# buckbaskin/parakeet_slam

Hardware: AMD Instinct MI355X
Metric: particle*landmark EKF updates/sec (whole filter step) (higher is better)
Workload: dtype f64

## Files before the change

include/parakeet_slam.h:

```cpp
#ifndef PARAKEET_SLAM_H_
#define PARAKEET_SLAM_H_

#include <stddef.h>
#include <stdint.h>

#ifdef __cplusplus
extern "C" {
#endif
#if defined(__GNUC__)
#pragma GCC visibility push(default)
#endif

#define PK_ABI_VERSION 1

typedef enum pk_status {
  PK_OK = 0,
  PK_ERR_INVALID = -1,
  PK_ERR_HIP = -2,
  PK_ERR_STATE = -3,
  PK_ERR_UNSUPPORTED = -4,
  PK_ERR_NOMEM = -5
} pk_status;

#define PK_LANDMARK_POTENTIAL 0x40000000
// ... 102 lines not shown
int pk_shard_adopt_local_dev(pk_filter* f, int32_t rank);
int pk_shard_adopt_remote_dev(pk_filter* f, int32_t rank, const void* dev_recv, int64_t n_received);
int pk_motion_range(pk_filter* f, double v, double w, double dt, uint64_t seed, uint64_t draw, int64_t p0, int64_t p1);
int pk_staged_takes_regs(pk_filter* f);
int pk_observe_staged_range(pk_filter* f, int32_t fresh, int64_t p0, int64_t p1, int32_t first, int32_t last);

int pk_shard_state_dev(pk_filter* f, double* dev_out);
int pk_shard_plan_balanced_dev(pk_filter* f, const double* dev_global_state, int64_t global_particles, const double* dev_gmax,
                               int32_t weight_domain, double u, int32_t world, int32_t rank, int64_t* dev_table);
int pk_shard_pack_balanced_dev(pk_filter* f, const int64_t* table, int32_t world, int32_t rank, void* dev_buf);
int pk_shard_adopt_balanced_dev(pk_filter* f, const int64_t* table, int32_t world, int32_t rank, const void* dev_recv,
                                int64_t n_received, int32_t mode);
int pk_shard_pack_balanced_loop_dev(pk_filter* f, int64_t keep, int64_t a0, int64_t a1, void* dev_buf);
int pk_shard_download_logical(pk_filter* f, int64_t* logical);
int pk_shard_upload_logical(pk_filter* f, const int64_t* logical);
int pk_shard_download_balanced_plan(pk_filter* f, int64_t* rel, int64_t* Hl, int32_t* alive);
int pk_shard_reset_placement(pk_filter* f);
int pk_shard_download_balanced_offspring(pk_filter* f, int64_t global_particles, int64_t* H);
int pk_shard_balanced_errors(pk_filter* f, int64_t* count);

#define PK_PROBE_LEN 79
int pk_probe(int32_t device, const double pose[3], const double mean[5], const double cov[25],
             const double blob[4], const double Qt[16], double* out);

int pk_enable_timing(pk_filter* f, int32_t mask);
int pk_reset_timings(pk_filter* f);
int pk_timings(pk_filter* f, double ms[PK_T_COUNT], int64_t launches[PK_T_COUNT]);
int pk_observe_bytes(const pk_filter* f, int32_t num_blobs, int64_t* algorithmic, int64_t* moved);
enum {
  PK_ROUTE_NONE = 0,
  PK_ROUTE_KNOWN_IDS = 1,
  PK_ROUTE_ML_GENERAL = 2,
  PK_ROUTE_ML_HANDOFF = 3,
  PK_ROUTE_ML_SWEEP = 4,
  PK_ROUTE_ML_FUSED = 5,
  PK_ROUTE_ML_REGS = 6,
  PK_ROUTE_DENSE = 8,
  PK_ROUTE_ML_PUB_BIG = 9,
};
int pk_observe_route(const pk_filter* f);
int pk_download_sources(pk_filter* f, int32_t* src);
int pk_observe_flagged(pk_filter* f, int64_t* flagged, int64_t* cand_overflow);
int pk_observe_retry_rows(pk_filter* f, int64_t* wanted, int64_t* capacity);
int pk_observe_published(pk_filter* f, int32_t* published);
int pk_observe_pub_stats(pk_filter* f, int64_t stats[6]);
int pk_observe_flags(pk_filter* f, uint8_t* flags);
// ... 16 lines not shown
```

parakeet_slam_amd/_lib.py:

```python
from __future__ import annotations

import ctypes as C
import os

import numpy as np

HERE = os.path.dirname(os.path.abspath(__file__))
LIB_PATH = os.path.join(HERE, "libparakeet_slam.so")

PK_OK = 0
PK_ERR_INVALID, PK_ERR_HIP, PK_ERR_STATE, PK_ERR_UNSUPPORTED, PK_ERR_NOMEM = -1, -2, -3, -4, -5
PK_WEIGHTS_LINEAR, PK_WEIGHTS_LOG = 0, 1
PK_LANDMARK_POTENTIAL = 0x40000000
PK_T_NAMES = ("motion", "assoc", "observe", "weights", "resample", "summary", "materialise")
PK_T_COUNT = len(PK_T_NAMES)
PK_PROBE_LEN = 79
PK_ABI_VERSION = 1

_dp = C.POINTER(C.c_double)
_ip = C.POINTER(C.c_int32)
_lp = C.POINTER(C.c_int64)
_bp = C.POINTER(C.c_uint8)
_h = C.c_void_p

# ... 48 lines not shown
    "pk_shard_adopt_dev": (C.c_int, [_h, C.c_int32, C.c_void_p, C.c_int64]),
    "pk_shard_local_span_dev": (C.c_int, [_h, C.c_void_p]),
    "pk_shard_adopt_local_dev": (C.c_int, [_h, C.c_int32]),
    "pk_shard_adopt_remote_dev": (C.c_int, [_h, C.c_int32, C.c_void_p, C.c_int64]),
    "pk_shard_state_dev": (C.c_int, [_h, C.c_void_p]),
    "pk_shard_plan_balanced_dev": (C.c_int, [_h, C.c_void_p, C.c_int64, C.c_void_p, C.c_int32, C.c_double, C.c_int32, C.c_int32,
                                             C.c_void_p]),
    "pk_shard_pack_balanced_dev": (C.c_int, [_h, _lp, C.c_int32, C.c_int32, C.c_void_p]),
    "pk_shard_adopt_balanced_dev": (C.c_int, [_h, _lp, C.c_int32, C.c_int32, C.c_void_p, C.c_int64, C.c_int32]),
    "pk_shard_pack_balanced_loop_dev": (C.c_int, [_h, C.c_int64, C.c_int64, C.c_int64, C.c_void_p]),
    "pk_shard_download_logical": (C.c_int, [_h, _lp]),
    "pk_shard_reset_placement": (C.c_int, [_h]),
    "pk_shard_upload_logical": (C.c_int, [_h, _lp]),
    "pk_shard_download_balanced_plan": (C.c_int, [_h, _lp, _lp, _ip]),
    "pk_shard_download_balanced_offspring": (C.c_int, [_h, C.c_int64, _lp]),
    "pk_shard_balanced_errors": (C.c_int, [_h, _lp]),
    "pk_motion_range": (C.c_int, [_h, C.c_double, C.c_double, C.c_double, C.c_uint64, C.c_uint64, C.c_int64, C.c_int64]),
    "pk_staged_takes_regs": (C.c_int, [_h]),
    "pk_observe_staged_range": (C.c_int, [_h, C.c_int32, C.c_int64, C.c_int64, C.c_int32, C.c_int32]),
    "pk_particle_bytes": (C.c_int64, [_h]),
    "pk_pack_particles": (C.c_int, [_h, _lp, C.c_int64, C.c_void_p]),
    "pk_adopt_particles": (C.c_int, [_h, _lp, C.c_void_p, C.c_int64]),
    "pk_probe": (C.c_int, [C.c_int32, _dp, _dp, _dp, _dp, _dp, _dp]),
    "pk_enable_timing": (C.c_int, [_h, C.c_int32]),
    "pk_reset_timings": (C.c_int, [_h]),
    "pk_timings": (C.c_int, [_h, _dp, _lp]),
    "pk_observe_bytes": (C.c_int, [_h, C.c_int32, _lp, _lp]),
    "pk_observe_route": (C.c_int, [_h]),
    "pk_download_sources": (C.c_int, [_h, _ip]),
    "pk_observe_flagged": (C.c_int, [_h, _lp, _lp]),
    "pk_observe_retry_rows": (C.c_int, [_h, _lp, _lp]),
    "pk_grow_enable": (C.c_int, [_h, C.c_int32, C.c_int32, C.c_double]),
    "pk_grow_download": (C.c_int, [_h, C.c_int64, C.c_int64, _ip, _dp, _ip]),
    "pk_grow_upload": (C.c_int, [_h, C.c_int64, C.c_int64, _ip, _dp, _ip]),
    "pk_grow_shape": (C.c_int, [_h, C.POINTER(C.c_int32), C.POINTER(C.c_int32), C.POINTER(C.c_int32)]),
    "pk_observe_published": (C.c_int, [_h, C.POINTER(C.c_int32)]),
    "pk_observe_flags": (C.c_int, [_h, _bp]),
    "pk_observe_pub_stats": (C.c_int, [_h, _lp]),
    "pk_rng_create_numpy": (C.c_int, [C.c_uint32, C.POINTER(_h)]),
    "pk_rng_create_python": (C.c_int, [C.c_uint32, C.POINTER(_h)]),
    "pk_rng_destroy": (C.c_int, [_h]),
    "pk_rng_standard_normal": (C.c_int, [_h, C.c_int64, _dp]),
    "pk_rng_random": (C.c_int, [_h, C.c_int64, _dp]),
}


# ... 390 lines not shown
        return {k: (float(ms[i]), int(n[i])) for i, k in enumerate(PK_T_NAMES)}

    def observe_bytes(self, num_blobs):
        a = C.c_int64()
        m = C.c_int64()
        check(self._lib.pk_observe_bytes(self._h, int(num_blobs), C.byref(a), C.byref(m)))
        return int(a.value), int(m.value)


def probe(pose, mean, cov, blob, Qt=None, device=0):
    lib = load()
    Qt = 0.1 * np.identity(4) if Qt is None else Qt
    out = np.empty(PK_PROBE_LEN, dtype=np.float64)
    check(lib.pk_probe(int(device), dptr(f64(pose, (3,))), dptr(f64(mean, (5,))), dptr(f64(cov, (25,))),
                       dptr(f64(blob, (4,))), dptr(f64(Qt, (16,))), dptr(out)))
    return dict(
        probability_of_match=out[0], prob_position_match=out[1], closest_point=out[2:4].copy(),
        prob_color_match=out[4], zhat=out[5:9].copy(), H0=out[9:11].copy(), Q=out[11:27].reshape(4, 4).copy(),
        K=out[27:47].reshape(5, 4).copy(), weight=out[47], new_mean=out[48:53].copy(),
        new_cov=out[53:78].reshape(5, 5).copy(), log_weight=out[78],
    )


class HostRng(object):

    def __init__(self, seed, kind="numpy"):
        self._lib = load()
        self._h = _h()
        fn = self._lib.pk_rng_create_numpy if kind == "numpy" else self._lib.pk_rng_create_python
        check(fn(int(seed) & 0xFFFFFFFF, C.byref(self._h)))

    def standard_normal(self, n):
        out = np.empty(int(n), dtype=np.float64)
        check(self._lib.pk_rng_standard_normal(self._h, int(n), dptr(out)))
        return out

    def random(self, n=None):
        out = np.empty(1 if n is None else int(n), dtype=np.float64)
        check(self._lib.pk_rng_random(self._h, out.size, dptr(out)))
        return float(out[0]) if n is None else out

    def __del__(self):
        try:
            if self._h.value:
                self._lib.pk_rng_destroy(self._h)
                self._h = _h()
# ... 3 lines not shown
```

parakeet_slam_amd/csrc/pk_api.hip:

```cpp
#include <hip/hip_runtime.h>

#include <cmath>
#include <cstdarg>
#include <cstdio>
#include <cstring>
#include <new>
#include <string>
#include <vector>

#include "../../include/parakeet_slam.h"
#include "pk_kernels.hpp"

using namespace pk;

extern "C" {
int pk_download_landmarks(pk_filter* f, int64_t p0, int64_t p1, double* means, double* covs, int32_t* counts);
int pk_upload_landmarks(pk_filter* f, int64_t p0, int64_t p1, const double* means, const double* covs, const int32_t* counts);
}

#ifdef PK_STAMPS
namespace pk { void debug_read_stamps(unsigned long long* out, bool reset); void debug_read_fused_stamps(unsigned long long* out, bool reset); void debug_read_regs_stamps(unsigned long long* out, bool reset); void debug_read_pub_stamps(unsigned long long* out, bool reset); void debug_read_pub_wave_stamps(unsigned long long* out, bool reset); }
#endif

namespace {
// ... 2605 lines not shown
  PK_HIP(hipSetDevice(device));
  double in[55];
  memcpy(in, pose, 3 * 8);
  memcpy(in + 3, mean, 5 * 8);
  memcpy(in + 8, cov, 25 * 8);
  memcpy(in + 33, blob, 4 * 8);
  memcpy(in + 37, Qt, 16 * 8);
  blob_directions(blob, 1, in + 53);
  double* dev = nullptr;
  PK_HIP(hipMalloc((void**)&dev, (55 + PK_PROBE_LEN) * sizeof(double)));
  hipError_t e = hipMemcpy(dev, in, sizeof(in), hipMemcpyHostToDevice);
  if (e == hipSuccess) {
    if (dense)
      launch_probe_dense(nullptr, dev, dev + 55);
    else
      launch_probe(nullptr, dev, dev + 55);
    e = hipMemcpy(out, dev + 55, PK_PROBE_LEN * sizeof(double), hipMemcpyDeviceToHost);
  }
  (void)hipFree(dev);
  if (e != hipSuccess) return fail(PK_ERR_HIP, "pk_probe: %s", hipGetErrorString(e));
  return PK_OK;
}

#ifdef PK_STAMPS
__attribute__((visibility("default"))) int pk_debug_pub_wave_stamps(unsigned long long* out, int reset) {
  pk::debug_read_pub_wave_stamps(out, reset != 0);
  return PK_OK;
}
__attribute__((visibility("default"))) int pk_debug_stamps(unsigned long long* out, int reset) {
  pk::debug_read_stamps(out, reset != 0);
  pk::debug_read_fused_stamps(out + 16, reset != 0);
  pk::debug_read_regs_stamps(out + 32, reset != 0);
  pk::debug_read_pub_stamps(out + 48, reset != 0);
  return PK_OK;
}
#endif

int pk_enable_timing(pk_filter* f, int32_t on) {
  if (!f) return fail(PK_ERR_INVALID, "pk_enable_timing: NULL handle");
  int rc;
  if ((rc = use_device(f))) return rc;
  if ((rc = drain_timings(f))) return rc;
  f->timing_mask = on < 0 ? 0xffffffffu : (uint32_t)on;
  return PK_OK;
}
int pk_reset_timings(pk_filter* f) {
// ... 106 lines not shown
```

parakeet_slam_amd/csrc/pk_device.hpp:

```cpp
#pragma once
#include <hip/hip_runtime.h>

#include <cfloat>
#include <climits>
#include <cstring>
#include <type_traits>

#include "pk_kernels.hpp"
#include "pk_math.hpp"

namespace pk {

constexpr int kWave = 64;
constexpr int kObsThreads = 256;
constexpr int kRedBlocks = 1024;

__device__ __forceinline__ void lds_barrier() { asm volatile("s_waitcnt lgkmcnt(0)\n\ts_barrier" ::: "memory"); }

#ifdef PK_STAMPS
#define PK_STAMP(var) \
  unsigned long long var; \
  asm volatile("s_memtime %0\n\ts_waitcnt lgkmcnt(0)" : "=s"(var)::"memory");
#else
#define PK_STAMP(var)
#endif

__device__ __forceinline__ double wave_sum(double v) {
#pragma unroll
  for (int off = 32; off > 0; off >>= 1) v += __shfl_xor(v, off, kWave);
  return v;
}
__device__ __forceinline__ double wave_max(double v) {
#pragma unroll
  for (int off = 32; off > 0; off >>= 1) v = fmax(v, __shfl_xor(v, off, kWave));
  return v;
}

template <int NW>
__device__ __forceinline__ double block_sum(double v, double* lds ) {
  v = wave_sum(v);
  const int wave = threadIdx.x / kWave, lane = threadIdx.x % kWave;
  __syncthreads();
  if (lane == 0) lds[wave] = v;
  __syncthreads();
  double t = lds[0];
#pragma unroll
  for (int i = 1; i < NW; ++i) t += lds[i];
  return t;
}
template <int NW>
__device__ __forceinline__ double block_sum_lds_only(double v, double* lds , int tid) {
  v = wave_sum(v);
// ... 96 lines not shown
```

parakeet_slam_amd/csrc/pk_k_motion.hip:

```cpp
#include "pk_device.hpp"
#include "pk_philox.hpp"

namespace pk {

__global__ void __launch_bounds__(256) k_motion(double* __restrict__ x, double* __restrict__ y,
                                                double* __restrict__ h, int64_t P, double v, double w,
                                                double dt, double sd, double sh,
                                                const double* __restrict__ z, uint64_t seed,
                                                uint64_t draw, int64_t goff, int motion_blocks,
                                                uint4* __restrict__ up_dst, const uint4* __restrict__ up_src,
                                                int64_t up_n16, const int64_t* __restrict__ logical,
                                                double* __restrict__ pose_part) {
  __shared__ double red[4];
  if ((int)blockIdx.x >= motion_blocks) {
    const int64_t nb = (int64_t)gridDim.x - motion_blocks;
    for (int64_t i = (int64_t)(blockIdx.x - motion_blocks) * blockDim.x + threadIdx.x; i < up_n16; i += nb * blockDim.x)
      up_dst[i] = up_src[i];
    return;
  }
  int64_t i = (int64_t)blockIdx.x * blockDim.x + threadIdx.x;
  if (i >= P && pose_part == nullptr) return;
  double px = 0.0, py = 0.0, ps = 0.0, pc = 0.0;
  if (i < P) {
  double z0, z1, z2;
// ... 226 lines not shown
  out[50] = g.mr;
  out[51] = g.mg;
  out[52] = g.mb;
  double* S = out + 53;
  S[0] = g.pxx;
  S[1] = g.pxy;
  S[5] = g.pxy;
  S[6] = g.pyy;
  S[12] = g.crr;
  S[13] = g.crg;
  S[14] = g.crb;
  S[17] = g.crg;
  S[18] = g.cgg;
  S[19] = g.cgb;
  S[22] = g.crb;
  S[23] = g.cgb;
  S[24] = g.cbb;
  out[78] = lw;
}
void launch_probe(hipStream_t s, const double* in_dev, double* out_dev) {
  hipLaunchKernelGGL(k_probe, dim3(1), dim3(64), 0, s, in_dev, out_dev);
}

}
```

parakeet_slam_amd/csrc/pk_k_step_pub.hip:

```cpp
#include <type_traits>

#include "pk_device.hpp"
#include "pk_pub_math.hpp"
#include "pk_pub_layout.hpp"

namespace pk {

#ifndef PK_PUB_ABLATE
#define PK_PUB_ABLATE 0
#endif

typedef double Double2 __attribute__((ext_vector_type(2)));
typedef int Int2 __attribute__((ext_vector_type(2)));

__device__ __forceinline__ double pose_scalar(const double* a, int64_t p) {
  return ((const __attribute__((address_space(4))) double*)a)[p];
}
__device__ __forceinline__ int32_t regs_source_pub(const int32_t* src, int64_t p) {
  return ((const __attribute__((address_space(4))) int32_t*)src)[p];
}

struct PubArgs {
  SlotSource ss;
  unsigned char* map_dst;
// ... 634 lines not shown
        for (int r = kMid; r < SLOTS; ++r) {
          contenders += v[h][r] < pub_inf() ? 1 : 0;
          close |= v[h][r] != best[h] && v[h][r] - best[h] < 1e-7;
        }
      }
      doubt |= close || (contenders >= 2 && best[h] > 1350.0);
    }
#pragma unroll
    for (int h = 0; h < TWO; ++h) {
      unsigned we = kRankMajor ? g[h] : offs[h] + wr[h];
      if constexpr (kRankMajor) we += wr[h] == 0u ? 0u : wr[h] == 1u ? G : rb[wr[h]];
      pub[best[h] < pub_inf() ? we : dump] = best[h] < pub_inf() ? pub_marker() : pub_inf();
    }
  }
  if (doubt) *flag = 1;
}

__device__ __forceinline__ void pub_take(PubSlots& q, const double* pub, unsigned dump) {
  const unsigned sw[kPubSlots] = {q.s[0], q.s[1], q.s[2], q.s[3]};
  double m[kPubSlots];
#pragma unroll
  for (int s = 0; s < kPubSlots; ++s) {
    const unsigned e = sw[s] >> 16;
    m[s] = pub[e == 0xFFFFu ? dump : e];
  }
#pragma unroll
  for (int s = 0; s < kPubSlots; ++s) {
    const unsigned e = sw[s] >> 16;
    const bool pos = ((q.st >> (4 * s)) & 1u) != 0u;
    if (pos && (e == 0xFFFFu || m[s] == pub_marker())) q.st |= 4u << (4 * s);
  }
}

#ifndef PK_DIAG_LOG_PER_UPDATE
#define PK_PROD_PTR(p_) (&(p_))
#else
#define PK_PROD_PTR(p_) ((double*)nullptr)
#endif
__device__ __forceinline__ void pub_fold_norms(double& acc, double& prod, bool last) {
#ifndef PK_DIAG_LOG_PER_UPDATE
  if (last || __ballot(!(prod > 1e-150 && prod < 1e150)) != 0ull) {
    acc -= 0.25 * log_few_ulp(prod);
    prod = 1.0;
  }
#else
  (void)acc;
  (void)prod;
// ... 122 lines not shown
  (void)hipDeviceSynchronize();
  (void)hipMemcpyFromSymbol(out, HIP_SYMBOL(pk_pstamp_acc), sizeof(unsigned long long) * 16);
  if (reset) {
    unsigned long long z[16] = {0};
    (void)hipMemcpyToSymbol(HIP_SYMBOL(pk_pstamp_acc), z, sizeof(z));
  }
}
#else
#define PK_PSTAMP(slot, a, b)
#endif

typedef const __attribute__((address_space(4))) PubArgs* PubArgsPtr;
__device__ __forceinline__ PubArgsPtr pub_args_now(PubArgsPtr rp) {
  asm volatile("" : "+s"(rp));
  return rp;
}
__device__ __forceinline__ SlotSource pub_slot_source(PubArgsPtr R) {
  return SlotSource{R->ss.map, R->ss.slot_bytes, R->ss.alt, R->ss.alt_stride, R->ss.alt_off};
}
__device__ __forceinline__ Noise<double> pub_noise(PubArgsPtr R) {
  return Noise<double>{R->qt.q00, R->qt.rr, R->qt.rg, R->qt.rb, R->qt.gg, R->qt.gb, R->qt.bb, R->qt.diag};
}

#ifdef PK_DIAG_NO_XCD_RUNS
__device__ __forceinline__ int64_t pub_walk_first(int64_t p_begin, int64_t) { return p_begin + blockIdx.x; }
__device__ __forceinline__ int64_t pub_walk_stride() { return (int64_t)gridDim.x; }
__device__ __forceinline__ int64_t pub_walk_limit(int64_t, int64_t p_end) { return p_end; }
#else
__device__ __forceinline__ int64_t pub_walk_first(int64_t p_begin, int64_t p_end) {
  const unsigned g = gridDim.x, b = blockIdx.x;
  if ((g & 7u) != 0u) return p_begin + b;
  const int64_t chunk = (p_end - p_begin + 7) / 8;
  return p_begin + (int64_t)(b & 7u) * chunk + (int64_t)(b >> 3);
}
__device__ __forceinline__ int64_t pub_walk_stride() { return (gridDim.x & 7u) != 0u ? (int64_t)gridDim.x : (int64_t)(gridDim.x >> 3); }
__device__ __forceinline__ int64_t pub_walk_limit(int64_t p_begin, int64_t p_end) {
  const unsigned g = gridDim.x, b = blockIdx.x;
  if ((g & 7u) != 0u) return p_end;
  const int64_t chunk = (p_end - p_begin + 7) / 8, e = p_begin + (int64_t)((b & 7u) + 1u) * chunk;
  return e < p_end ? e : p_end;
}
#endif
template <int NP, int THREADS>
__global__ void __launch_bounds__(THREADS, THREADS == 256 ? 3 : 1) k_step_pub(PubArgs a_unused) {
  constexpr int kPubThreads = THREADS, kPubWaves = THREADS / kWave;
  extern __shared__ __align__(16) unsigned char smem[];
  __shared__ double red[2][kPubWaves];
  __shared__ int wg_flag[2];
  constexpr bool kPerm = NP == 2 && THREADS == 512;
  __shared__ unsigned short s_perm[kPerm ? 2 * kPubOctets : 1];
  __shared__ unsigned s_rb[kCandSlots];
  constexpr int kUnmWords = THREADS == kPubSmallThreads ? 32 : 96;
  __shared__ unsigned s_ubits[kUnmWords];
#define PK_PUB_L0(q_, t_) (!kPerm ? 2 * kPubThreads * (q_) + 2 * (t_) : (int)(((lw >> (16 + 8 * (q_))) & 0xFFu) << 4) + 2 * ((t_)&7))
  PubArgsPtr rp = (PubArgsPtr)__builtin_amdgcn_kernarg_segment_ptr();
  const int tid0 = threadIdx.x;
  int B, Lp, L, ecap;
  {
    PubArgsPtr R = pub_args_now(rp);
    if (*R->skip != 0u) return;
    B = R->B;
    Lp = R->Lp;
    L = R->L;
    ecap = R->ecap;
  }
  const unsigned Bp = ((unsigned)B + 15u) & ~15u;
  const unsigned o_pub = Bp * 48u, o_binfo = o_pub + ((unsigned)ecap + 2u) * 8u, o_order = o_binfo + Bp * 4u, o_any = o_order + Bp * 2u;
  const unsigned o_imm = o_any + 2u * (Bp + 16u);
  const unsigned o_bnd = o_imm + (unsigned)kPubImmBytes;
  const unsigned dump = (unsigned)ecap, anydump = Bp;
  unsigned G;
  {
    const int tid = tid0;
    PubArgsPtr R = pub_args_now(rp);
    {
      const uint4* gf = R->far;
      float2* bnd = reinterpret_cast<float2*>(smem + o_bnd);
      for (int i = tid; i < Lp; i += kPubThreads) {
        float2 v = make_float2(-3.0e38f, 0.f);
        if (gf) {
          const uint4 hdr = gf[2 * (size_t)i];
          if (hdr.z != 0u) v = make_float2(__uint_as_float(hdr.x), __uint_as_float(hdr.y));
        }
        bnd[i] = v;
      }
    }
    double* ex = reinterpret_cast<double*>(smem);
    const double* gex = R->exact;
// ... 3 lines not shown
    const unsigned* gb = R->glist;
    const unsigned short* go = R->order;
    G = gb[B];
    for (int i = tid; i < B; i += kPubThreads) {
      glist[i] = (unsigned)i < G ? gb[i] : 0u;
      order[i] = go[i];
    }
    for (unsigned i = (unsigned)tid; i < 2u * (Bp + 16u) / 4u; i += kPubThreads) reinterpret_cast<unsigned*>(smem + o_any)[i] = 0u;
    const unsigned char* gi = R->immutable;
    for (int i = tid; i < Lp; i += kPubThreads) smem[o_imm + (unsigned)i] = i < L ? gi[i] : (unsigned char)0;
    if constexpr (kPerm) {
      if (tid < 2 * kPubOctets) s_perm[tid] = reinterpret_cast<const unsigned short*>(gb + B + 1)[tid];
    }
    if (tid < kCandSlots) s_rb[tid] = gb[B + 1 + kPubTailWords + tid];
    for (int i = tid; i < kUnmWords; i += kPubThreads) s_ubits[i] = 0u;
    if (tid == 0) {
      wg_flag[0] = 0;
      wg_flag[1] = 0;
    }
  }
  __syncthreads();

  int64_t prev = -1;
  int cur = 0;
  int32_t nsrc;
  {
    PubArgsPtr R = pub_args_now(rp);
    const int64_t p0 = pub_walk_first(R->p_begin, R->P), pl = pub_walk_limit(R->p_begin, R->P);
    nsrc = regs_source_pub(R->src, p0 < pl ? p0 : pl - 1);
  }
#ifdef PK_STAMPS
  unsigned long long pst[12] = {0, 0, 0, 0, 0, 0, 0, 0, 0, 0, 0, 0};
#endif
#define PK_PUB_ROW(q_, field, F)                                                                  \
  {                                                                                               \
    const Double2 v_ = *reinterpret_cast<const Double2*>(sf_ + (size_t)F * Lp + lbq_);            \
    S[2 * (q_)].field = v_.x;                                                                     \
    S[2 * (q_) + 1].field = v_.y;                                                                 \
  }
#define PK_PUB_LOAD_MEANS(q_, sslot_, lb_)                                                        \
  {                                                                                               \
    const double* sf_ = reinterpret_cast<const double*>(sslot_);                                  \
    const int lbq_ = (lb_);                                                                       \
    PK_PUB_ROW(q_, mx, F_MX)                                                                      \
    PK_PUB_ROW(q_, my, F_MY)                                                                      \
    PK_PUB_ROW(q_, mr, F_MR)                                                                      \
// ... 70 lines not shown
      tid = (int)(lw & 0xFFFFu);
    }
    double* ex = reinterpret_cast<double*>(smem);
    double* pub = reinterpret_cast<double*>(smem + o_pub);
    const unsigned* glist = reinterpret_cast<const unsigned*>(smem + o_binfo);
    const unsigned short* order = reinterpret_cast<const unsigned short*>(smem + o_order);
    unsigned char* anyc = smem + o_any + (unsigned)cur * (Bp + 16u);
    PubSlots Q[2 * NP];
    double pse[2 * NP];
    bool done;
    PK_STAMP(s0)
#ifdef PK_STAMPS
    unsigned long long s3 = s0;
#endif
    {
      PubArgsPtr R = pub_args_now(rp);
      const int64_t Pn = pub_walk_limit(R->p_begin, R->P);
      done = p >= Pn;
      const int64_t pc = done ? Pn - 1 : p;
      {
        const SlotSource ss = pub_slot_source(R);
        const unsigned char* sslot = ss.at(nsrc);
        const double sx = pose_scalar(R->x, pc), sy = pose_scalar(R->y, pc), sh = pose_scalar(R->h, pc);
        int lbase[NP];
#pragma unroll
        for (int q = 0; q < NP; ++q) lbase[q] = min(PK_PUB_L0(q, tid), Lp - 2);
        uint4 cref[2 * NP], ccw[2 * NP], cew[2 * NP];
        auto request_cand = [&](int q) {
          PubArgsPtr R2 = pub_args_now(rp);
#ifdef PK_DIAG_TAIL_LISTS
          const int lc = lbase[q];
#else
          const int lc = min(PK_PUB_L0(q, tid), Lp);
#endif
          const uint4* cr = R2->cand + 2 * (size_t)lc;
          const uint4* er = R2->erec + lc;
          cref[2 * q] = cr[0];
          ccw[2 * q] = cr[1];
          cref[2 * q + 1] = cr[2];
          ccw[2 * q + 1] = cr[3];
          cew[2 * q] = er[0];
          cew[2 * q + 1] = er[1];
        };
        request_cand(0);
        asm volatile("" ::: "memory");
        {
// ... 84 lines not shown
        if (!done) {
          do_pair(std::integral_constant<int, 0>{});
          if constexpr (NP > 1) {
            PK_PUB_LOAD_MEANS(1, sslot, lbase[1])
            request_cand(NP - 1);
            {
              asm volatile("" ::: "memory");
              PubArgsPtr R7 = pub_args_now(rp);
              PK_PUB_LOAD_COVS(1, sslot, R7->count_off, lbase[1])
            }
            do_pair(std::integral_constant<int, 1>{});
          }
        }
        PK_STAMP(s2)
        PK_PSTAMP(1, s1, s2)
#ifdef PK_STAMPS
        s3 = s2;
#endif
      }
    }
    lds_barrier();
    PK_STAMP(s4)
    PK_PSTAMP(3, s3, s4)
    if (prev >= 0 && tid == 0) {
      PubArgsPtr R = pub_args_now(rp);
      double tot = red[cur ^ 1][0];
#pragma unroll
      for (int i = 1; i < kPubWaves; ++i) tot += red[cur ^ 1][i];
      double* logw = R->logw;
      const double w = (R->reset ? 0.0 : logw[prev]) + tot;
      logw[prev] = w;
      unsigned long long* gk = R->gmax_key;
      if (gk) atomicMax(gk + (prev & (kGmaxKeys - 1)), double_to_key(w));
      R->src[prev] = (int32_t)prev;
    }
    if (done) break;
    prev = -1;
    double acc;
    {
      int nun = 0;
      for (unsigned w = (unsigned)tid; w < Bp / 4u; w += kPubThreads) {
        const unsigned v = reinterpret_cast<const unsigned*>(anyc)[w];
#pragma unroll
        for (int b = 0; b < 4; ++b) nun += ((int)(4 * w + b) < B && ((v >> (8 * b)) & 0xFFu) == 0u) ? 1 : 0;
      }
      acc = (double)nun * Consts<double>::log_no_match;
      unsigned* anyn = reinterpret_cast<unsigned*>(smem + o_any + (unsigned)(cur ^ 1) * (Bp + 16u));
      for (unsigned w = (unsigned)tid; w < Bp / 4u; w += kPubThreads) anyn[w] = 0u;
      if (tid == 0) wg_flag[cur ^ 1] = 0;
    }
    if (pub_args_now(rp)->unm != nullptr) pub_note_unmatched<THREADS>(tid, anyc, order, B, Bp, s_ubits);
    if (PK_PUB_ABLATE < 2) pub_settle_blobs<THREADS>(tid, glist, G, pub, dump, &wg_flag[cur], s_rb);
    PK_STAMP(s5)
    PK_PSTAMP(4, s4, s5)
    lds_barrier();
    {
      PubArgsPtr Ru = pub_args_now(rp);
      if (Ru->unm != nullptr) pub_store_unmatched<THREADS>(tid, s_ubits, Ru->unm + (size_t)p * Ru->unm_words, Ru->unm_words);
    }
#pragma unroll
    for (int i = 0; i < 2 * NP; ++i)
      if (PK_PUB_ABLATE < 2) pub_take(Q[i], pub, dump);
    lds_barrier();
    PK_STAMP(s6)
    PK_PSTAMP(5, s5, s6)
    if (wg_flag[cur] && PK_PUB_ABLATE == 0) {
      if (tid == 0) {
        PubArgsPtr R = pub_args_now(rp);
        R->pflag_out[p] = 1;
        atomicAdd(R->n_flagged, 1u);
      }
      {
        PubArgsPtr R6 = pub_args_now(rp);
        const unsigned char* ns = pub_slot_source(R6).at(nsrc);
        const int coff = R6->count_off;
#pragma unroll
        for (int q = 0; q < kPipe; ++q) PK_PUB_LOAD_PAIR(q, ns, coff, min(PK_PUB_L0(q, tid), Lp - 2))
      }
      continue;
    }
    {
      PubArgsPtr R = pub_args_now(rp);
      if (tid == 0) R->pflag_out[p] = 0;
      const Noise<double> qt = pub_noise(R);
      const double sx = pose_scalar(R->x, p), sy = pose_scalar(R->y, p);
      unsigned char* dslot = R->map_dst + (size_t)p * R->ss.slot_bytes;
      double* df = reinterpret_cast<double*>(dslot);
      int* dc = reinterpret_cast<int*>(dslot + R->count_off);
// ... 168 lines not shown

#define PK_BIG_FIRST(R_) pub_walk_first((R_)->p_begin, (R_)->P)
#define PK_BIG_STRIDE() pub_walk_stride()
#define PK_BIG_LIMIT(R_) pub_walk_limit((R_)->p_begin, (R_)->P)
template <int NCH>
__global__ void __launch_bounds__(kPubThreads) k_step_pub_big(PubArgs a_unused) {
  extern __shared__ __align__(16) unsigned char smem[];
  __shared__ double red[2][kPubThreads / kWave];
  __shared__ int wg_flag[2];
  __shared__ unsigned short s_bperm[kPubBigPlaces];
  __shared__ unsigned s_rb[kPubBigSlots];
  __shared__ unsigned s_novf[2];
  __shared__ unsigned s_ubits[kPubUnmWords];
#define PK_BIG_L0(q_, t_) ((int)(16u * (unsigned)s_bperm[kPubOctets * (q_) + ((t_) >> 3)]) + 2 * ((t_)&7))
  constexpr int kPubWaves = kPubThreads / kWave;
#ifdef PK_DIAG_BIG_FRONT_TO_BACK
  constexpr bool kBack = false;
#else
  constexpr bool kBack = NCH < 6;
#endif
  PubArgsPtr rp = (PubArgsPtr)__builtin_amdgcn_kernarg_segment_ptr();
  const int tid0 = threadIdx.x;
  int B, Lp, L, ecap;
  {
    PubArgsPtr R = pub_args_now(rp);
    if (*R->skip != 0u) return;
    B = R->B;
    Lp = R->Lp;
    L = R->L;
    ecap = R->ecap;
  }
  const unsigned Bp = ((unsigned)B + 15u) & ~15u;
  const unsigned o_glist = ((unsigned)ecap + 2u) * 8u, o_any = o_glist + Bp * 4u;
  const unsigned dump = (unsigned)ecap, anydump = Bp;
  unsigned G;
  unsigned ovf0, n_places;
  {
    const int tid = tid0;
    PubArgsPtr R = pub_args_now(rp);
    unsigned* glist = reinterpret_cast<unsigned*>(smem + o_glist);
    const unsigned* gb = R->glist;
    G = gb[B];
    const unsigned E = R->stats[0];
    ovf0 = (E + 1u) & ~1u;
    n_places = (unsigned)ecap > ovf0 ? ((unsigned)ecap - ovf0) / 2u : 0u;
    if (n_places > 0xFFFEu) n_places = 0xFFFEu;
    for (int i = tid; i < B; i += kPubThreads) glist[i] = (unsigned)i < G ? gb[i] : 0u;
    for (unsigned i = (unsigned)tid; i < 2u * (Bp + 16u) / 4u; i += kPubThreads) reinterpret_cast<unsigned*>(smem + o_any)[i] = 0u;
    if (tid < kPubBigPlaces) s_bperm[tid] = reinterpret_cast<const unsigned short*>(gb + B + 1)[2 * kPubOctets + tid];
    if (tid < kPubBigSlots) s_rb[tid] = gb[B + 1 + kPubTailWords + tid];
    for (int i = tid; i < kPubUnmWords; i += kPubThreads) s_ubits[i] = 0u;
    if (tid == 0) {
      wg_flag[0] = 0;
      wg_flag[1] = 0;
// ... 17 lines not shown
    PK_BIG_LOAD(SA, SB, mb, F_MB, lb_)                                                                \
    asm volatile("" ::: "memory");                                                                    \
    PK_BIG_LOAD(SA, SB, pxx, F_PXX, lb_)                                                              \
    PK_BIG_LOAD(SA, SB, pxy, F_PXY, lb_)                                                              \
    PK_BIG_LOAD(SA, SB, pyy, F_PYY, lb_)                                                              \
    PK_BIG_LOAD(SA, SB, crr, F_CRR, lb_)                                                              \
    PK_BIG_LOAD(SA, SB, crg, F_CRG, lb_)                                                              \
    PK_BIG_LOAD(SA, SB, crb, F_CRB, lb_)                                                              \
    PK_BIG_LOAD(SA, SB, cgg, F_CGG, lb_)                                                              \
    PK_BIG_LOAD(SA, SB, cgb, F_CGB, lb_)                                                              \
    PK_BIG_LOAD(SA, SB, cbb, F_CBB, lb_)                                                              \
    const Int2 c_ = *reinterpret_cast<const Int2*>(sc_ + (lb_));                                      \
    SA.count = c_.x;                                                                                  \
    SB.count = c_.y;                                                                                  \
    asm volatile("" ::: "memory");                                                                    \
  }
#define PK_BIG_LOAD(SA, SB, field, F, lb_)                                                            \
  {                                                                                                   \
    const Double2 v_ = *reinterpret_cast<const Double2*>(sf_ + (size_t)F * Lp + (lb_));              \
    SA.field = v_.x;                                                                                  \
    SB.field = v_.y;                                                                                  \
  }
  int64_t prev = -1;
  int cur = 0;
#ifdef PK_STAMPS
  unsigned long long pst[12] = {0, 0, 0, 0, 0, 0, 0, 0, 0, 0, 0, 0};
#define PK_BIG_WAIT_ALL asm volatile("s_waitcnt vmcnt(0)" ::: "memory");
#else
#define PK_BIG_WAIT_ALL
#endif
  int32_t nsrc;
  {
    PubArgsPtr R = pub_args_now(rp);
    const int64_t p0 = PK_BIG_FIRST(R), pl = PK_BIG_LIMIT(R);
    nsrc = regs_source_pub(R->src, p0 < pl ? p0 : pl - 1);
  }
  Landmark<double> SA, SB;
  {
    const int lb0 = min(PK_BIG_L0(0, tid0), Lp - 2);
    PK_BIG_ROWS(SA, SB, lb0, nsrc)
  }
  for (int64_t p = PK_BIG_FIRST(pub_args_now(rp));; p += PK_BIG_STRIDE(), cur ^= 1) {
    int tid = tid0;
    asm volatile("" : "+v"(tid));
    const int32_t csrc = nsrc;
    double* pub = reinterpret_cast<double*>(smem);
    const unsigned* glist = reinterpret_cast<const unsigned*>(smem + o_glist);
    unsigned char* anyc = smem + o_any + (unsigned)cur * (Bp + 16u);
    PubSlots Q[2 * NCH];
    double pse[2 * NCH];
#pragma unroll
    for (int i = 0; i < 2 * NCH; ++i) {
      Q[i] = kPubNoSlots;
      pse[i] = 0.0;
    }
    bool done;
    {
      PubArgsPtr R = pub_args_now(rp);
      done = p >= PK_BIG_LIMIT(R);
    }
    PK_STAMP(b0)
    if (!done) {
#pragma unroll 1
      for (int q = 0; q < NCH; ++q) {
        PubSlots qa = kPubNoSlots, qb = kPubNoSlots;
        double pa = 0.0, pb = 0.0;
        if (2 * kPubThreads * q < Lp) {
          const int l0 = PK_BIG_L0(q, tid);
          PubArgsPtr R = pub_args_now(rp);
          PK_STAMP(c0)
          const double sx = pose_scalar(R->x, p), sy = pose_scalar(R->y, p), sh = pose_scalar(R->h, p);
#ifdef PK_DIAG_TAIL_LISTS
          const int lc = min(l0, Lp - 2);
#else
          const int lc = min(l0, Lp);
#endif
          const uint4* cr = R->cand + 3 * (size_t)lc;
          const uint4* er = R->erec + 2 * (size_t)lc;
          PubGateIn gi[2];
          gi[0].ref = cr[0];
          gi[0].cw[0] = cr[1];
          gi[1].ref = cr[3];
// ... 119 lines not shown
            pse[i] = pse[i - 2];
          }
          Q[0] = qa;
          Q[1] = qb;
          pse[0] = pa;
          pse[1] = pb;
        } else {
#pragma unroll
          for (int i = 0; i + 2 < 2 * NCH; ++i) {
            Q[i] = Q[i + 2];
            pse[i] = pse[i + 2];
          }
          Q[2 * NCH - 2] = qa;
          Q[2 * NCH - 1] = qb;
          pse[2 * NCH - 2] = pa;
          pse[2 * NCH - 1] = pb;
        }
      }
    }
    PK_STAMP(b1)
    lds_barrier();
    PK_STAMP(b2)
    PK_PSTAMP(4, b1, b2)
    if (prev >= 0 && tid == 0) {
      PubArgsPtr R = pub_args_now(rp);
      double tot = red[cur ^ 1][0];
#pragma unroll
      for (int i = 1; i < kPubWaves; ++i) tot += red[cur ^ 1][i];
      double* logw = R->logw;
      const double w = (R->reset ? 0.0 : logw[prev]) + tot;
      logw[prev] = w;
      unsigned long long* gk = R->gmax_key;
      if (gk) atomicMax(gk + (prev & (kGmaxKeys - 1)), double_to_key(w));
      R->src[prev] = (int32_t)prev;
    }
    if (done) break;
    prev = -1;
    double acc;
    {
      int nun = 0;
      for (unsigned w = (unsigned)tid; w < Bp / 4u; w += kPubThreads) {
        const unsigned v = reinterpret_cast<const unsigned*>(anyc)[w];
#pragma unroll
        for (int b = 0; b < 4; ++b) nun += ((int)(4 * w + b) < B && ((v >> (8 * b)) & 0xFFu) == 0u) ? 1 : 0;
      }
      acc = (double)nun * Consts<double>::log_no_match;
      unsigned* anyn = reinterpret_cast<unsigned*>(smem + o_any + (unsigned)(cur ^ 1) * (Bp + 16u));
      for (unsigned w = (unsigned)tid; w < Bp / 4u; w += kPubThreads) anyn[w] = 0u;
      if (tid == 0) {
        wg_flag[cur ^ 1] = 0;
        s_novf[cur ^ 1] = 0u;
      }
    }
    {
      PubArgsPtr Ru = pub_args_now(rp);
      if (Ru->unm != nullptr) pub_note_unmatched<kPubThreads>(tid, anyc, Ru->order, B, Bp, s_ubits);
    }
    pub_settle_blobs<kPubThreads, kPubBigSlots>(tid, glist, G, pub, dump, &wg_flag[cur], s_rb);
    lds_barrier();
    PK_STAMP(b3)
    PK_PSTAMP(5, b2, b3)
    {
      PubArgsPtr Ru = pub_args_now(rp);
      if (Ru->unm != nullptr) pub_store_unmatched<kPubThreads>(tid, s_ubits, Ru->unm + (size_t)p * Ru->unm_words, Ru->unm_words);
    }
#pragma unroll
    for (int i = 0; i < 2 * NCH; ++i) pub_take(Q[i], pub, dump);
    if (s_novf[cur] != 0u) {
#pragma unroll
      for (int i = 0; i < 2 * NCH; ++i) pub_take_parked(Q[i], reinterpret_cast<const uint4*>(smem) + ovf0 / 2u, pub, dump, &wg_flag[cur]);
    }
    lds_barrier();
    PK_STAMP(b4)
    PK_PSTAMP(6, b3, b4)
    if (wg_flag[cur]) {
      if (tid == 0) {
        PubArgsPtr R = pub_args_now(rp);
        R->pflag_out[p] = 1;
        atomicAdd(R->n_flagged, 1u);
      }
      {
        const int lb0 = min(PK_BIG_L0(0, tid), Lp - 2);
        PK_BIG_ROWS(SA, SB, lb0, nsrc)
      }
      continue;
    }
    if (tid == 0) pub_args_now(rp)->pflag_out[p] = 0;
#define PK_BIG_STORE(field, F)                                                             \
  {                                                                                        \
    const Double2 v_ = {SA.field, SB.field};                                               \
    __builtin_nontemporal_store(v_, reinterpret_cast<Double2*>(df + (size_t)F * Lp + l0)); \
  }
    double nprod = 1.0;
#pragma unroll 1
    for (int qr = 0; qr < NCH; ++qr) {
      const int q = kBack ? NCH - 1 - qr : qr;
      if (2 * kPubThreads * q < Lp) {
// ... 206 lines not shown
```

parakeet_slam_amd/csrc/pk_kernels.hpp:

```cpp
#pragma once
#include <hip/hip_runtime.h>

#include <cstdint>

#include "pk_layout.hpp"

namespace pk {

struct NoiseD {
  double q00, rr, rg, rb, gg, gb, bb;
};

struct DeviceState {
  int64_t P;
  MapLayout lay;
  double* x[2];
  double* y[2];
  double* h[2];
  double* logw[2];
  int32_t* src[2];
  int cur;
  unsigned char* map[2];
  int mcur;
  unsigned char* immutable;
// ... 185 lines not shown
size_t step_pub_duo_lds_bytes(int B, const DuoLimits& lim);
void launch_step_pub_duo(hipStream_t s, DeviceState& d, int B, const double* exact_dev, const unsigned short* order_dev,
                         const FastHandoff& fh, const NoiseD& qt, const ObserveExtras& ex, const CandTable& cand, const uint4* erec_dev,
                         const unsigned* glist_dev, const unsigned* skip_duo_dev, const unsigned* stats_dev, const DuoLimits& lim,
                         const float4* gate4_dev, const uint4* prim_dev, int64_t p0 = 0, int64_t p1 = -1, int reserve_cus = 0);
extern int g_observe_nv;
inline size_t observe_general_lds_bytes(int Lp, int B) { return sizeof(int32_t) * ((size_t)Lp + 2 * (size_t)B); }
inline size_t assoc_brute_lds_bytes(int B) { return (size_t)B * 12; }
void launch_block_max(hipStream_t s, DeviceState& d, double* partial_dev, double* gmax_dev);
void launch_keys_max(hipStream_t s, const unsigned long long* keys_dev, double* gmax_dev);
void launch_scan_local(hipStream_t s, DeviceState& d, const double* gmax_dev, int domain,
                       double* clocal_dev, double* totals_dev, const unsigned long long* gmax_key_dev = nullptr);
void launch_scan_blocks(hipStream_t s, const double* totals_dev, int64_t nb, double* offsets_dev,
                        double* sum_dev);
constexpr int64_t kAncestorsScanMaxBlocks = 256;
void launch_ancestors(hipStream_t s, const double* clocal_dev, const double* totals_dev,
                      const double* offsets_dev, const double* sum_dev, int64_t nb, int64_t P_global,
                      int64_t P_scan, double u, int64_t slot0, int64_t n, int32_t* anc_dev,
                      DeviceState* gather = nullptr);
void launch_summary_partials(hipStream_t s, DeviceState& d, double* partial_dev, double* out4_dev);
void launch_materialise(hipStream_t s, DeviceState& d);
void launch_broadcast_slot(hipStream_t s, DeviceState& d, const unsigned char* slot_dev);
void launch_probe(hipStream_t s, const double* in_dev, double* out_dev);
size_t dense_lds_bytes(int Lp, int B);
void launch_observe_dense(hipStream_t s, DeviceState& d, const double* blobs_dev, const double* blobdir_dev, int B,
                          const int32_t* ids_in_dev, int32_t* ids_out_dev, const double Qt[16], bool update,
                          const ObserveExtras& ex);
void launch_probe_dense(hipStream_t s, const double* in_dev, double* out_dev);
constexpr size_t kPoseRecordBytes = 8 * sizeof(double);
struct BalancedBuffers {
  double* glogw = nullptr;
  double* clocal = nullptr;
  double* totals = nullptr;
  double* offsets = nullptr;
  double* sum = nullptr;
  int64_t* H = nullptr;
  long long* cloc = nullptr;
  long long* ctot = nullptr;
  long long* coff = nullptr;
  int64_t* rel = nullptr;
  int64_t* Hl = nullptr;
  int32_t* alive = nullptr;
  int* bad = nullptr;
  int64_t cap = 0;
};
void launch_iota64(hipStream_t s, int64_t* p, int64_t n, int64_t off);
// ... 34 lines not shown
```

Measured before the change: 26.45 billion.

## Use permlane/DPP wave reduction and trim per-particle reloads in publish kernels

Replaces the shuffle-based double wave_sum with permlane32/16 swaps plus DPP row operations, avoiding LDS-backed shuffles. The publish kernels now skip the pub reads in pub_take when no lane in the wave needs them. They cache the unmatched-pointer check instead of reloading kernel arguments, and move the previous particle's log-weight load earlier so it overlaps other work. A probe entry point is added to test the new reduction, and the DPP control values and lane semantics carry correctness risk.

```diff
diff --git a/include/parakeet_slam.h b/include/parakeet_slam.h
--- a/include/parakeet_slam.h
+++ b/include/parakeet_slam.h
@@ -148,6 +148,7 @@
 #define PK_PROBE_LEN 79
 int pk_probe(int32_t device, const double pose[3], const double mean[5], const double cov[25],
              const double blob[4], const double Qt[16], double* out);
+int pk_probe_wave_sum(int32_t device, const double* in, int32_t rows, double* out);
 
 int pk_enable_timing(pk_filter* f, int32_t mask);
 int pk_reset_timings(pk_filter* f);
diff --git a/parakeet_slam_amd/_lib.py b/parakeet_slam_amd/_lib.py
--- a/parakeet_slam_amd/_lib.py
+++ b/parakeet_slam_amd/_lib.py
@@ -94,6 +94,7 @@
     "pk_pack_particles": (C.c_int, [_h, _lp, C.c_int64, C.c_void_p]),
     "pk_adopt_particles": (C.c_int, [_h, _lp, C.c_void_p, C.c_int64]),
     "pk_probe": (C.c_int, [C.c_int32, _dp, _dp, _dp, _dp, _dp, _dp]),
+    "pk_probe_wave_sum": (C.c_int, [C.c_int32, _dp, C.c_int32, _dp]),
     "pk_enable_timing": (C.c_int, [_h, C.c_int32]),
     "pk_reset_timings": (C.c_int, [_h]),
     "pk_timings": (C.c_int, [_h, _dp, _lp]),
@@ -530,6 +531,16 @@
     )
 
 
+def probe_wave_sum(rows, device=0):
+    lib = load()
+    a = np.ascontiguousarray(rows, dtype=np.float64)
+    if a.ndim != 2 or a.shape[1] != 64:
+        raise ValueError("probe_wave_sum: rows of 64 doubles, got shape %r" % (a.shape,))
+    out = np.empty_like(a)
+    check(lib.pk_probe_wave_sum(int(device), dptr(a), int(a.shape[0]), dptr(out)))
+    return out
+
+
 class HostRng(object):
 
     def __init__(self, seed, kind="numpy"):
diff --git a/parakeet_slam_amd/csrc/pk_api.hip b/parakeet_slam_amd/csrc/pk_api.hip
--- a/parakeet_slam_amd/csrc/pk_api.hip
+++ b/parakeet_slam_amd/csrc/pk_api.hip
@@ -2651,6 +2651,27 @@
   return PK_OK;
 }
 
+int pk_probe_wave_sum(int32_t device, const double* in, int32_t rows, double* out) {
+  if (!in || !out) return fail(PK_ERR_INVALID, "pk_probe_wave_sum: NULL argument");
+  if (rows <= 0 || rows > 65536) return fail(PK_ERR_INVALID, "pk_probe_wave_sum: %d rows", rows);
+  int ndev = pk_device_count();
+  if (ndev <= 0) return fail(PK_ERR_HIP, "pk_probe_wave_sum: no HIP device visible (the HIP path has no CPU fallback)");
+  if (device < 0 || device >= ndev) return fail(PK_ERR_INVALID, "pk_probe_wave_sum: device %d of %d", device, ndev);
+  PK_HIP(hipSetDevice(device));
+  const size_t n = (size_t)rows * 64;
+  double* dev = nullptr;
+  PK_HIP(hipMalloc((void**)&dev, 2 * n * sizeof(double)));
+  hipError_t e = hipMemcpy(dev, in, n * sizeof(double), hipMemcpyHostToDevice);
+  if (e == hipSuccess) {
+    launch_probe_wave_sum(nullptr, dev, dev + n, rows);
+    e = hipGetLastError();
+  }
+  if (e == hipSuccess) e = hipMemcpy(out, dev + n, n * sizeof(double), hipMemcpyDeviceToHost);
+  (void)hipFree(dev);
+  if (e != hipSuccess) return fail(PK_ERR_HIP, "pk_probe_wave_sum: %s", hipGetErrorString(e));
+  return PK_OK;
+}
+
 #ifdef PK_STAMPS
 __attribute__((visibility("default"))) int pk_debug_pub_wave_stamps(unsigned long long* out, int reset) {
   pk::debug_read_pub_wave_stamps(out, reset != 0);
diff --git a/parakeet_slam_amd/csrc/pk_device.hpp b/parakeet_slam_amd/csrc/pk_device.hpp
--- a/parakeet_slam_amd/csrc/pk_device.hpp
+++ b/parakeet_slam_amd/csrc/pk_device.hpp
@@ -25,9 +25,35 @@
 #define PK_STAMP(var)
 #endif
 
+typedef unsigned UInt2 __attribute__((ext_vector_type(2)));
+template <int CTRL>
+__device__ __forceinline__ double wave_dpp(double v) {
+  const int l = __builtin_amdgcn_update_dpp(0, __double2loint(v), CTRL, 0xF, 0xF, true);
+  const int h = __builtin_amdgcn_update_dpp(0, __double2hiint(v), CTRL, 0xF, 0xF, true);
+  return __hiloint2double(h, l);
+}
 __device__ __forceinline__ double wave_sum(double v) {
+#ifdef PK_DIAG_SHFL_WAVE_SUM
 #pragma unroll
   for (int off = 32; off > 0; off >>= 1) v += __shfl_xor(v, off, kWave);
+#else
+  {
+    const unsigned lo = (unsigned)__double2loint(v), hi = (unsigned)__double2hiint(v);
+    const UInt2 a = __builtin_amdgcn_permlane32_swap(lo, lo, false, false);
+    const UInt2 b = __builtin_amdgcn_permlane32_swap(hi, hi, false, false);
+    v = __hiloint2double((int)b.x, (int)a.x) + __hiloint2double((int)b.y, (int)a.y);
+  }
+  {
+    const unsigned lo = (unsigned)__double2loint(v), hi = (unsigned)__double2hiint(v);
+    const UInt2 a = __builtin_amdgcn_permlane16_swap(lo, lo, false, false);
+    const UInt2 b = __builtin_amdgcn_permlane16_swap(hi, hi, false, false);
+    v = __hiloint2double((int)b.x, (int)a.x) + __hiloint2double((int)b.y, (int)a.y);
+  }
+  v += wave_dpp<0x128>(v);
+  v += wave_dpp<0x1B>(wave_dpp<0x141>(v));
+  v += wave_dpp<0x4E>(v);
+  v += wave_dpp<0xB1>(v);
+#endif
   return v;
 }
 __device__ __forceinline__ double wave_max(double v) {
diff --git a/parakeet_slam_amd/csrc/pk_k_motion.hip b/parakeet_slam_amd/csrc/pk_k_motion.hip
--- a/parakeet_slam_amd/csrc/pk_k_motion.hip
+++ b/parakeet_slam_amd/csrc/pk_k_motion.hip
@@ -272,4 +272,12 @@
   hipLaunchKernelGGL(k_probe, dim3(1), dim3(64), 0, s, in_dev, out_dev);
 }
 
-}
+__global__ void __launch_bounds__(kWave) k_probe_wave_sum(const double* __restrict__ in, double* __restrict__ out) {
+  const size_t i = (size_t)blockIdx.x * kWave + threadIdx.x;
+  out[i] = wave_sum(in[i]);
+}
+void launch_probe_wave_sum(hipStream_t s, const double* in_dev, double* out_dev, int rows) {
+  hipLaunchKernelGGL(k_probe_wave_sum, dim3(rows), dim3(kWave), 0, s, in_dev, out_dev);
+}
+
+}
diff --git a/parakeet_slam_amd/csrc/pk_k_step_pub.hip b/parakeet_slam_amd/csrc/pk_k_step_pub.hip
--- a/parakeet_slam_amd/csrc/pk_k_step_pub.hip
+++ b/parakeet_slam_amd/csrc/pk_k_step_pub.hip
@@ -680,7 +680,13 @@
 #pragma unroll
   for (int s = 0; s < kPubSlots; ++s) {
     const unsigned e = sw[s] >> 16;
+#ifdef PK_DIAG_TAKE_READS_ALL
     m[s] = pub[e == 0xFFFFu ? dump : e];
+#else
+    const bool need = ((q.st >> (4 * s)) & 1u) != 0u && e != 0xFFFFu;
+    m[s] = 0.0;
+    if (__ballot(need) != 0ull) m[s] = pub[e == 0xFFFFu ? dump : e];
+#endif
   }
 #pragma unroll
   for (int s = 0; s < kPubSlots; ++s) {
@@ -849,6 +855,21 @@
   return Noise<double>{R->qt.q00, R->qt.rr, R->qt.rg, R->qt.rb, R->qt.gg, R->qt.gb, R->qt.bb, R->qt.diag};
 }
 
+template <int NW>
+__device__ __forceinline__ void pub_finish_weight(PubArgsPtr R, const double* redp, int64_t prev, double lw_old) {
+  double tot = redp[0];
+#pragma unroll
+  for (int i = 1; i < NW; ++i) tot += redp[i];
+  const double w = lw_old + tot;
+  R->logw[prev] = w;
+  unsigned long long* gk = R->gmax_key;
+  if (gk) atomicMax(gk + (prev & (kGmaxKeys - 1)), double_to_key(w));
+  R->src[prev] = (int32_t)prev;
+}
+__device__ __forceinline__ double pub_weight_before(PubArgsPtr R, int64_t p) {
+  return R->reset ? 0.0 : pose_scalar(R->logw, p);
+}
+
 #ifdef PK_DIAG_NO_XCD_RUNS
 __device__ __forceinline__ int64_t pub_walk_first(int64_t p_begin, int64_t) { return p_begin + blockIdx.x; }
 __device__ __forceinline__ int64_t pub_walk_stride() { return (int64_t)gridDim.x; }
@@ -883,6 +904,7 @@
   PubArgsPtr rp = (PubArgsPtr)__builtin_amdgcn_kernarg_segment_ptr();
   const int tid0 = threadIdx.x;
   int B, Lp, L, ecap;
+  bool has_unm;
   {
     PubArgsPtr R = pub_args_now(rp);
     if (*R->skip != 0u) return;
@@ -890,7 +912,9 @@
     Lp = R->Lp;
     L = R->L;
     ecap = R->ecap;
-  }
+    has_unm = R->unm != nullptr;
+  }
+  (void)has_unm;
   const unsigned Bp = ((unsigned)B + 15u) & ~15u;
   const unsigned o_pub = Bp * 48u, o_binfo = o_pub + ((unsigned)ecap + 2u) * 8u, o_order = o_binfo + Bp * 4u, o_any = o_order + Bp * 2u;
   const unsigned o_imm = o_any + 2u * (Bp + 16u);
@@ -940,6 +964,7 @@
   __syncthreads();
 
   int64_t prev = -1;
+  double lw_prev = 0.0;
   int cur = 0;
   int32_t nsrc;
   {
@@ -1056,6 +1081,9 @@
         const SlotSource ss = pub_slot_source(R);
         const unsigned char* sslot = ss.at(nsrc);
         const double sx = pose_scalar(R->x, pc), sy = pose_scalar(R->y, pc), sh = pose_scalar(R->h, pc);
+#ifndef PK_DIAG_WEIGHT_AT_A
+        if (prev >= 0) lw_prev = pub_weight_before(R, prev);
+#endif
         int lbase[NP];
 #pragma unroll
         for (int q = 0; q < NP; ++q) lbase[q] = min(PK_PUB_L0(q, tid), Lp - 2);
@@ -1186,6 +1214,7 @@
     lds_barrier();
     PK_STAMP(s4)
     PK_PSTAMP(3, s3, s4)
+#ifdef PK_DIAG_WEIGHT_AT_A
     if (prev >= 0 && tid == 0) {
       PubArgsPtr R = pub_args_now(rp);
       double tot = red[cur ^ 1][0];
@@ -1200,6 +1229,12 @@
     }
     if (done) break;
     prev = -1;
+#else
+    if (done) {
+      if (prev >= 0 && tid == 0) pub_finish_weight<kPubWaves>(pub_args_now(rp), red[cur ^ 1], prev, lw_prev);
+      break;
+    }
+#endif
     double acc;
     {
       int nun = 0;
@@ -1213,21 +1248,36 @@
       for (unsigned w = (unsigned)tid; w < Bp / 4u; w += kPubThreads) anyn[w] = 0u;
       if (tid == 0) wg_flag[cur ^ 1] = 0;
     }
+#ifdef PK_DIAG_UNM_RELOADS
     if (pub_args_now(rp)->unm != nullptr) pub_note_unmatched<THREADS>(tid, anyc, order, B, Bp, s_ubits);
+#else
+    if (has_unm) pub_note_unmatched<THREADS>(tid, anyc, order, B, Bp, s_ubits);
+#endif
     if (PK_PUB_ABLATE < 2) pub_settle_blobs<THREADS>(tid, glist, G, pub, dump, &wg_flag[cur], s_rb);
     PK_STAMP(s5)
     PK_PSTAMP(4, s4, s5)
     lds_barrier();
+#ifdef PK_DIAG_UNM_RELOADS
     {
       PubArgsPtr Ru = pub_args_now(rp);
       if (Ru->unm != nullptr) pub_store_unmatched<THREADS>(tid, s_ubits, Ru->unm + (size_t)p * Ru->unm_words, Ru->unm_words);
     }
+#else
+    if (has_unm) {
+      PubArgsPtr Ru = pub_args_now(rp);
+      pub_store_unmatched<THREADS>(tid, s_ubits, Ru->unm + (size_t)p * Ru->unm_words, Ru->unm_words);
+    }
+#endif
 #pragma unroll
     for (int i = 0; i < 2 * NP; ++i)
       if (PK_PUB_ABLATE < 2) pub_take(Q[i], pub, dump);
     lds_barrier();
     PK_STAMP(s6)
     PK_PSTAMP(5, s5, s6)
+#ifndef PK_DIAG_WEIGHT_AT_A
+    if (prev >= 0 && tid == 0) pub_finish_weight<kPubWaves>(pub_args_now(rp), red[cur ^ 1], prev, lw_prev);
+    prev = -1;
+#endif
     if (wg_flag[cur] && PK_PUB_ABLATE == 0) {
       if (tid == 0) {
         PubArgsPtr R = pub_args_now(rp);
@@ -1442,6 +1492,7 @@
   PubArgsPtr rp = (PubArgsPtr)__builtin_amdgcn_kernarg_segment_ptr();
   const int tid0 = threadIdx.x;
   int B, Lp, L, ecap;
+  bool has_unm;
   {
     PubArgsPtr R = pub_args_now(rp);
     if (*R->skip != 0u) return;
@@ -1449,7 +1500,9 @@
     Lp = R->Lp;
     L = R->L;
     ecap = R->ecap;
-  }
+    has_unm = R->unm != nullptr;
+  }
+  (void)has_unm;
   const unsigned Bp = ((unsigned)B + 15u) & ~15u;
   const unsigned o_glist = ((unsigned)ecap + 2u) * 8u, o_any = o_glist + Bp * 4u;
   const unsigned dump = (unsigned)ecap, anydump = Bp;
@@ -1513,6 +1566,7 @@
     SB.field = v_.y;                                                                                  \
   }
   int64_t prev = -1;
+  double lw_prev = 0.0;
   int cur = 0;
 #ifdef PK_STAMPS
   unsigned long long pst[12] = {0, 0, 0, 0, 0, 0, 0, 0, 0, 0, 0, 0};
@@ -1549,6 +1603,9 @@
     {
       PubArgsPtr R = pub_args_now(rp);
       done = p >= PK_BIG_LIMIT(R);
+#ifndef PK_DIAG_WEIGHT_AT_A
+      if (prev >= 0) lw_prev = pub_weight_before(R, prev);
+#endif
     }
     PK_STAMP(b0)
     if (!done) {
@@ -1714,6 +1771,7 @@
     lds_barrier();
     PK_STAMP(b2)
     PK_PSTAMP(4, b1, b2)
+#ifdef PK_DIAG_WEIGHT_AT_A
     if (prev >= 0 && tid == 0) {
       PubArgsPtr R = pub_args_now(rp);
       double tot = red[cur ^ 1][0];
@@ -1728,6 +1786,12 @@
     }
     if (done) break;
     prev = -1;
+#else
+    if (done) {
+      if (prev >= 0 && tid == 0) pub_finish_weight<kPubWaves>(pub_args_now(rp), red[cur ^ 1], prev, lw_prev);
+      break;
+    }
+#endif
     double acc;
     {
       int nun = 0;
@@ -1744,18 +1808,29 @@
         s_novf[cur ^ 1] = 0u;
       }
     }
+#ifdef PK_DIAG_UNM_RELOADS
     {
       PubArgsPtr Ru = pub_args_now(rp);
       if (Ru->unm != nullptr) pub_note_unmatched<kPubThreads>(tid, anyc, Ru->order, B, Bp, s_ubits);
     }
+#else
+    if (has_unm) pub_note_unmatched<kPubThreads>(tid, anyc, pub_args_now(rp)->order, B, Bp, s_ubits);
+#endif
     pub_settle_blobs<kPubThreads, kPubBigSlots>(tid, glist, G, pub, dump, &wg_flag[cur], s_rb);
     lds_barrier();
     PK_STAMP(b3)
     PK_PSTAMP(5, b2, b3)
+#ifdef PK_DIAG_UNM_RELOADS
     {
       PubArgsPtr Ru = pub_args_now(rp);
       if (Ru->unm != nullptr) pub_store_unmatched<kPubThreads>(tid, s_ubits, Ru->unm + (size_t)p * Ru->unm_words, Ru->unm_words);
     }
+#else
+    if (has_unm) {
+      PubArgsPtr Ru = pub_args_now(rp);
+      pub_store_unmatched<kPubThreads>(tid, s_ubits, Ru->unm + (size_t)p * Ru->unm_words, Ru->unm_words);
+    }
+#endif
 #pragma unroll
     for (int i = 0; i < 2 * NCH; ++i) pub_take(Q[i], pub, dump);
     if (s_novf[cur] != 0u) {
@@ -1765,6 +1840,10 @@
     lds_barrier();
     PK_STAMP(b4)
     PK_PSTAMP(6, b3, b4)
+#ifndef PK_DIAG_WEIGHT_AT_A
+    if (prev >= 0 && tid == 0) pub_finish_weight<kPubWaves>(pub_args_now(rp), red[cur ^ 1], prev, lw_prev);
+    prev = -1;
+#endif
     if (wg_flag[cur]) {
       if (tid == 0) {
         PubArgsPtr R = pub_args_now(rp);
diff --git a/parakeet_slam_amd/csrc/pk_kernels.hpp b/parakeet_slam_amd/csrc/pk_kernels.hpp
--- a/parakeet_slam_amd/csrc/pk_kernels.hpp
+++ b/parakeet_slam_amd/csrc/pk_kernels.hpp
@@ -231,6 +231,7 @@
 void launch_materialise(hipStream_t s, DeviceState& d);
 void launch_broadcast_slot(hipStream_t s, DeviceState& d, const unsigned char* slot_dev);
 void launch_probe(hipStream_t s, const double* in_dev, double* out_dev);
+void launch_probe_wave_sum(hipStream_t s, const double* in_dev, double* out_dev, int rows);
 size_t dense_lds_bytes(int Lp, int B);
 void launch_observe_dense(hipStream_t s, DeviceState& d, const double* blobs_dev, const double* blobdir_dev, int B,
                           const int32_t* ids_in_dev, int32_t* ids_out_dev, const double Qt[16], bool update,
```

Measured after the change: 26.50 billion (median of 3 runs). About the same (+0.2%).
